# Sahar-E/NeRF-and-DietNeRF

Hardware: AMD Instinct MI355X
Metric: rays/sec (coarse+fine) at 256x256, 64 coarse + 128 fine samples (higher is better)
Workload: dtype f16 (3-pass hi/lo split operands, f32 accumulate; fp32-class results)

## Files before the change

### include/nerf_mi355.h

```cpp
#ifndef NERF_MI355_H
#define NERF_MI355_H

#include <stddef.h>
#include <stdint.h>

#ifdef __cplusplus
extern "C" {
#endif

#define NERF_ABI_VERSION 6

enum { NERF_NET_COARSE = 0, NERF_NET_FINE = 1 };
enum { NERF_MEM_HOST = 0, NERF_MEM_DEVICE = 1 };
enum {
    NERF_PRECISION_FP32 = 0,
    NERF_PRECISION_F16X3 = 1,
    NERF_PRECISION_F16 = 2,
    NERF_PRECISION_BF16X3 = 3
};

enum {
    NERF_SAMPLING_LINEAR = 0,
    NERF_SAMPLING_LINDISP = 1
};
// ... 133 lines not shown
                         uint64_t seed, float* grad_coarse, float* grad_fine, float* metrics, int mem);
int nerf_train_apply(nerf_ctx* ctx, const float* grad_coarse, const float* grad_fine, int mem);
int nerf_train_render_gradients(nerf_ctx* ctx, const float* rays_orig, const float* rays_dirs, const float* d_rgb,
                                int64_t N, int32_t Sc, int32_t Sf, const float* u_coarse, const float* u_fine,
                                uint64_t seed, int64_t ray_base, int32_t accumulate, float* rgb_out,
                                float* grad_coarse, float* grad_fine, int mem);
int nerf_train_render_forward(nerf_ctx* ctx, int32_t slot, const float* rays_orig, const float* rays_dirs, int64_t N,
                              int32_t Sc, int32_t Sf, const float* u_coarse, const float* u_fine, uint64_t seed,
                              int64_t ray_base, float* rgb_out, int mem);
int nerf_train_render_backward(nerf_ctx* ctx, int32_t slot, const float* d_rgb, int32_t accumulate, float* grad_coarse,
                               float* grad_fine, int mem);
int nerf_train_render_release(nerf_ctx* ctx);
int nerf_train_get_gradients(nerf_ctx* ctx, int which, float* blob, size_t n_floats, int mem);
int nerf_get_weights(nerf_ctx* ctx, int which, float* blob, size_t n_floats, int mem);

int nerf_ctx_enable_timing(nerf_ctx* ctx, int on);
int nerf_ctx_read_timing(nerf_ctx* ctx, double* mlp_ms, int64_t* n_launches, int64_t* n_rows);
int nerf_ctx_read_culling_timing(nerf_ctx* ctx, double* ms4, int64_t* n_passes);

#ifdef __cplusplus
}
#endif
#endif
```

### nerf_and_dietnerf_amd/_lib.py

```python
from __future__ import annotations

import ctypes as C
import os

_HERE = os.path.dirname(os.path.abspath(__file__))
LIB_PATH = os.environ.get("NERF_MI355_LIB") or os.path.join(_HERE, "lib", "libnerf_mi355.so")

NERF_NET_COARSE, NERF_NET_FINE = 0, 1
NERF_MEM_HOST, NERF_MEM_DEVICE = 0, 1
NERF_PRECISION_FP32, NERF_PRECISION_F16X3, NERF_PRECISION_F16, NERF_PRECISION_BF16X3 = 0, 1, 2, 3
NERF_SAMPLING_LINEAR, NERF_SAMPLING_LINDISP = 0, 1
NERF_RAYS_WORLD, NERF_RAYS_NDC = 0, 1
NERF_ABI_VERSION = 6


class NerfConfig(C.Structure):
    _fields_ = [
        ("n_pos_enc_xyz", C.c_int32), ("n_pos_enc_dir", C.c_int32), ("n_angles", C.c_int32),
        ("hidden_dim", C.c_int32), ("last_hidden_dim", C.c_int32), ("leaky_relu_alpha", C.c_float),
        ("near_boundary", C.c_float), ("far_boundary", C.c_float), ("precision", C.c_int32),
        ("device", C.c_int32),
    ]


# ... 65 lines not shown
    ("nerf_train_set_distortion_weights", C.c_int, [_P, _F, _F]),
    ("nerf_train_read_distortion_sums", C.c_int, [_P, C.POINTER(C.c_double), C.POINTER(_I64)]),
    ("nerf_distortion_loss", C.c_int, [_P, _P, _P, _I64, _I32, _P, _P, _P, C.c_int]),
    ("nerf_train_loss_scale", C.c_int, [_P, C.POINTER(C.c_float), C.POINTER(_I64), C.POINTER(_I64)]),
    ("nerf_train_read_metric_sums", C.c_int, [_P, C.POINTER(C.c_double), C.POINTER(_I64)]),
    ("nerf_train_step", C.c_int, [_P, _P, _P, _P, _I64, _I32, _I32, _P, _P, _U64, _P, C.c_int]),
    ("nerf_train_gradients", C.c_int, [_P, _P, _P, _P, _I64, _I32, _I32, _P, _P, _U64, _P, _P, _P, C.c_int]),
    ("nerf_train_apply", C.c_int, [_P, _P, _P, C.c_int]),
    ("nerf_train_render_gradients", C.c_int, [_P, _P, _P, _P, _I64, _I32, _I32, _P, _P, _U64, _I64, _I32, _P, _P, _P,
                                              C.c_int]),
    ("nerf_train_render_forward", C.c_int, [_P, _I32, _P, _P, _I64, _I32, _I32, _P, _P, _U64, _I64, _P, C.c_int]),
    ("nerf_train_render_backward", C.c_int, [_P, _I32, _P, _I32, _P, _P, C.c_int]),
    ("nerf_train_render_release", C.c_int, [_P]),
    ("nerf_train_get_gradients", C.c_int, [_P, C.c_int, _P, C.c_size_t, C.c_int]),
    ("nerf_get_weights", C.c_int, [_P, C.c_int, _P, C.c_size_t, C.c_int]),
    ("nerf_ctx_enable_timing", C.c_int, [_P, C.c_int]),
    ("nerf_ctx_read_timing", C.c_int, [_P, C.POINTER(C.c_double), C.POINTER(_I64), C.POINTER(_I64)]),
]

_lib = None


def load():
    global _lib
    if _lib is not None:
        return _lib
    if not os.path.exists(LIB_PATH):
        raise RuntimeError(
            f"{LIB_PATH} is missing: build the HIP extension first "
            "(python -c 'import __graft_entry__ as g; g.build()' or make -C nerf_and_dietnerf_amd/csrc). "
# ... 24 lines not shown
```

### nerf_and_dietnerf_amd/csrc/nerf_api.hip

```cpp
#include "../../include/nerf_mi355.h"

#include <stdarg.h>
#include <stdio.h>
#include <stdlib.h>
#include <string.h>

#include <algorithm>
#include <cmath>
#include <string>
#include <vector>

#include "nerf_ctx.h"

using namespace nerf;

thread_local std::string g_err;

namespace nerf {

int fail(const char* fmt, ...) {
    char buf[512];
    va_list ap;
    va_start(ap, fmt);
    vsnprintf(buf, sizeof buf, fmt, ap);
    va_end(ap);
    g_err = buf;
// ... 50 lines not shown
    return 0;
}

int enter(nerf_ctx* c) {
    if (!c) return fail("ctx is NULL");
    HIP_OK(hipSetDevice(c->cfg.device));
    return 0;
}

int sampling_ok(const nerf_ctx* c) {
    if (c->sampling == NERF_SAMPLING_LINDISP && !(c->cfg.near_boundary > 0.f)) return fail("lindisp needs near_boundary > 0");
    return 0;
}

int draw_z_values(nerf_ctx* c, const float* o, const float* d, long long N, int S, const float* u, uint64_t seed,
                  long long ray_base, float* z) {
    const float* bounds = nullptr;
    const int* state = nullptr;
    if (c->box_on && c->grid_R > 0 && o && d && N > 0) {
        if (int r = ensure(c, c->b_gbounds, (size_t)N * 8)) return r;
        if (int r = ensure(c, c->b_gstate, (size_t)N * 4)) return r;
        launch_ray_grid_bounds(c->box, c->cfg.near_boundary, c->cfg.far_boundary, (const uint32_t*)c->b_grid[c->grid_cur].p,
                               c->grid_R, o, d, N, (float*)c->b_gbounds.p, (int*)c->b_gstate.p, c->stream);
        bounds = (const float*)c->b_gbounds.p;
        state = (const int*)c->b_gstate.p;
    }
    launch_z_values(c->cfg.near_boundary, c->cfg.far_boundary, c->sampling == NERF_SAMPLING_LINDISP, N, S, u, seed, ray_base,
                    z, c->stream, o, d, c->box_on ? &c->box : nullptr, bounds, state);
    return 0;
}

static int cull_stamp(nerf_ctx* c, bool stamp = true) {
    if (!stamp || !c->timing) return 0;
    if (c->cull_ev_used == c->cull_ev.size()) {
        hipEvent_t e;
        HIP_OK(hipEventCreate(&e));
        c->cull_ev.push_back(e);
    }
    HIP_OK(hipEventRecord(c->cull_ev[c->cull_ev_used++], c->stream));
    return 0;
}

int compact_samples(nerf_ctx* c, SampleCompaction& rec, const float* o, const float* d, const float* z, long long N, int S,
// ... 112 lines not shown
    if (!cfg) return fail("nerf_config is NULL");
    if (cfg->n_angles != 2 && cfg->n_angles != 1 && cfg->n_angles != 0)
        return fail("n_angles_for_model should be 1 or 2.");
    if (cfg->n_pos_enc_xyz < 1 || cfg->n_pos_enc_xyz > kLxWide || cfg->n_pos_enc_dir < 1 || cfg->n_pos_enc_dir > kLd ||
        cfg->hidden_dim != kHidden || cfg->last_hidden_dim != kLast)
        return fail("supported networks: n_pos_enc_dim_xyz 1..%d, n_pos_enc_view_dir 1..%d, hidden %d, last hidden %d "
                    "(got %d %d %d %d)", kLxWide, kLd, kHidden, kLast, cfg->n_pos_enc_xyz, cfg->n_pos_enc_dir, cfg->hidden_dim,
                    cfg->last_hidden_dim);
    RenderKernel k;
    if (pick_render_kernel(*cfg, cfg->precision, false, &k) == 2)
        return fail("unknown precision %d (NERF_PRECISION_FP32 = 0, NERF_PRECISION_F16X3 = 1, NERF_PRECISION_F16 = 2, "
                    "NERF_PRECISION_BF16X3 = 3)", cfg->precision);
    return 0;
}

int run_mlp(nerf_ctx* c, int which, const RenderKernel& k, const float* in_a, const float* in_b, const float* z, float* raw,
            long long M, int S, int mode) {
    if (!c->net[which].loaded) return fail("network %d has no weights loaded", which);
    if (int r = train_flush_weights(c, which)) return r;
    MlpArgs a{};
    a.wstream = (const float*)c->net[which].stream[k.stream];
    a.wconst = c->net[which].cst[k.cst];
    if (!a.wstream || !a.wconst) return fail("internal: network %d keeps no stream of kind %d", which, (int)k.stream);
    a.in_a = in_a; a.in_b = in_b; a.z = z; a.raw = raw; a.M = M; a.S = S; a.mode = mode;
    a.nonfinite = c->nonfinite;
    a.alpha = c->cfg.leaky_relu_alpha;
    hipEvent_t e0 = nullptr, e1 = nullptr;
    if (c->timing) {
        if (c->ev_used == c->ev_pool.size()) {
            hipEvent_t x, y;
            HIP_OK(hipEventCreate(&x));
            HIP_OK(hipEventCreate(&y));
            c->ev_pool.emplace_back(x, y);
        }
        e0 = c->ev_pool[c->ev_used].first; e1 = c->ev_pool[c->ev_used].second;
        c->ev_used++;
        c->timed_rows += M;
        HIP_OK(hipEventRecord(e0, c->stream));
    }
    k.launch(a, c->num_cus, c->stream, c->cfg.n_angles == 0);
    if (c->timing) HIP_OK(hipEventRecord(e1, c->stream));
    HIP_OK(hipGetLastError());
    return 0;
}

struct OutSizes { size_t per_ray[7]; };
OutSizes out_sizes(int S) {
    OutSizes o;
    o.per_ray[0] = 3; o.per_ray[1] = S; o.per_ray[2] = S; o.per_ray[3] = S; o.per_ray[4] = 3 * (size_t)S;
    o.per_ray[5] = S; o.per_ray[6] = 1;
    return o;
}
float** out_ptrs(nerf_outputs& o, int i) {
    switch (i) {
        case 0: return &o.rgb; case 1: return &o.weights; case 2: return &o.cumprod; case 3: return &o.alpha;
        case 4: return &o.rgb_samples; case 5: return &o.z; default: return &o.depth;
    }
}

nerf_outputs stage_outputs(nerf_ctx* c, Staging& st, const nerf_outputs& outs, long long N, int S) {
    const OutSizes sz = out_sizes(S);
    nerf_outputs dev = outs;
    for (int i = 0; i < 7; ++i) {
        float** p = out_ptrs(dev, i);
        *p = st.out(c->b_out[i], *p, sz.per_ray[i] * N * sizeof(float));
    }
    return dev;
}

int copy_back_batch(nerf_ctx* c, const nerf_outputs* host, const nerf_outputs* dev, long long off, long long n, int S,
                    size_t batch_index) {
    if (!c->copy_stream) HIP_OK(hipStreamCreateWithFlags(&c->copy_stream, hipStreamNonBlocking));
    constexpr size_t kRing = 64;
    if (c->copy_ev.size() < kRing) {
        hipEvent_t e;
        HIP_OK(hipEventCreateWithFlags(&e, hipEventDisableTiming));
        c->copy_ev.push_back(e);
    }
    hipEvent_t ev = c->copy_ev[batch_index % c->copy_ev.size()];
    HIP_OK(hipEventRecord(ev, c->stream));
    HIP_OK(hipStreamWaitEvent(c->copy_stream, ev, 0));
    const OutSizes sz = out_sizes(S);
    nerf_outputs h = host ? *host : nerf_outputs{};
    nerf_outputs d = *dev;
    for (int i = 0; i < 7; ++i) {
        float* hp = *out_ptrs(h, i);
        if (!hp) continue;
        HIP_OK(hipMemcpyAsync(hp + sz.per_ray[i] * off, *out_ptrs(d, i) + sz.per_ray[i] * off,
                              sz.per_ray[i] * n * sizeof(float), hipMemcpyDeviceToHost, c->copy_stream));
    }
    return 0;
}

int culled_mlp(nerf_ctx* c, int which, const RenderKernel& k, const float* o, const float* d, const float* z, long long N, int S,
               float* raw) {
    if (!c->net[which].loaded) return fail("network %d has no weights loaded", which);
    if (int r = compact_samples(c, c->cull, o, d, z, N, S, true)) return r;
    const long long M = c->cull.rows;
    if (M > 0) {
        if (int r = ensure(c, c->b_craw, (size_t)M * (k.sigma_only ? 4 : 16))) return r;
        const float* view = c->cfg.n_angles != 0 ? (const float*)c->b_cdirs.p : nullptr;
        if (int r = run_mlp(c, which, k, (const float*)c->b_cxyz.p, view, nullptr, (float*)c->b_craw.p, M, 1, 1)) return r;
    }
    if (int r = cull_stamp(c)) return r;
    launch_raw_expand((const float*)c->b_craw.p, N * S, k.sigma_only, (const uint8_t*)c->cull.mask.p,
                      (const uint32_t*)c->cull.first.p, raw, c->stream);
    return cull_stamp(c);
}

int network_pass(nerf_ctx* c, int which, const RenderKernel& k, const float* o, const float* d, const float* z, long long N, int S,
                 float* raw) {
    if (!(culling_acts(c, c->cull_on) && N > 0)) return run_mlp(c, which, k, o, d, z, raw, N * S, S, 0);
    const size_t ev0 = c->cull_ev_used;
    const int r = culled_mlp(c, which, k, o, d, z, N, S, raw);
    if (r) c->cull_ev_used = ev0;
    return r;
}

int dev_render_rays(nerf_ctx* c, int which, const float* o, const float* d, const float* z, long long N, int S,
                    const nerf_outputs& outs) {
    const bool weights_only = outs.weights && !outs.rgb && !outs.cumprod && !outs.alpha && !outs.rgb_samples && !outs.z &&
                              !outs.depth;
    RenderKernel k;
    if (pick_render_kernel(c->cfg, c->cfg.precision, which == NERF_NET_COARSE && weights_only, &k)) return 1;
    if (k.sigma_only) {
        if (int r = ensure(c, c->b_raw, (size_t)N * S * sizeof(float))) return r;
        float* sigma = (float*)c->b_raw.p;
        if (int r = network_pass(c, which, k, o, d, z, N, S, sigma)) return r;
        launch_composite_weights(sigma, z, N, S, outs.weights, c->stream);
        HIP_OK(hipGetLastError());
        return 0;
    }
    if (int r = ensure(c, c->b_raw, (size_t)N * S * 4 * sizeof(float))) return r;
    float* raw = (float*)c->b_raw.p;
    if (int r = network_pass(c, which, k, o, d, z, N, S, raw)) return r;
    launch_composite(raw, z, N, S, outs.rgb, outs.weights, outs.cumprod, outs.alpha, outs.rgb_samples, outs.depth,
                     c->stream);
    if (outs.z && outs.z != z)
        HIP_OK(hipMemcpyAsync(outs.z, z, (size_t)N * S * sizeof(float), hipMemcpyDeviceToDevice, c->stream));
    HIP_OK(hipGetLastError());
    return 0;
}

int dev_render(nerf_ctx* c, const float* o, const float* d, long long N, int Sc, int Sf, const float* u_c,
               const float* u_f, uint64_t seed, long long ray_base, const nerf_outputs& outs) {
    const bool fine = Sf > 0 && c->net[NERF_NET_FINE].loaded;
    if (int r = sampling_ok(c)) return r;
    if (int r = ensure(c, c->b_zc, (size_t)N * Sc * sizeof(float))) return r;
    float* zc = (float*)c->b_zc.p;
    if (int r = draw_z_values(c, o, d, N, Sc, u_c, seed, ray_base, zc)) return r;
    if (!fine) return dev_render_rays(c, NERF_NET_COARSE, o, d, zc, N, Sc, outs);
    if (Sc < 2) return fail("hierarchical sampling needs at least 2 coarse samples (got %d)", Sc);
    if (int r = ensure(c, c->b_wc, (size_t)N * Sc * sizeof(float))) return r;
    nerf_outputs co{};
    co.weights = (float*)c->b_wc.p;
    if (int r = dev_render_rays(c, NERF_NET_COARSE, o, d, zc, N, Sc, co)) return r;
    const int St = Sc + Sf;
    if (int r = ensure(c, c->b_zf, (size_t)N * St * sizeof(float))) return r;
    float* zf = (float*)c->b_zf.p;
    launch_sample_pdf(co.weights, zc, N, Sc, Sf, u_f, seed, ray_base, nullptr, zf, c->stream);
    return dev_render_rays(c, NERF_NET_FINE, o, d, zf, N, St, outs);
}

}

extern "C" {

int nerf_abi_version(void) { return NERF_ABI_VERSION; }
const char* nerf_last_error(void) { return g_err.c_str(); }

size_t nerf_blob_size(const nerf_config* cfg) {
    if (check_cfg(cfg)) return 0;
    return blob_floats(cfg->n_pos_enc_xyz, cfg->n_pos_enc_dir, cfg->n_angles);
}

int nerf_ctx_create(const nerf_config* cfg, nerf_ctx** out) {
// ... 32 lines not shown
    bf16::wide::mlp_bf16x3_set_attributes();
    mlp_bwd_f16x3_set_attributes();
    mlp_f16_2t_set_attributes();
    *out = c;
    return 0;
}

void nerf_ctx_destroy(nerf_ctx* c) {
    if (!c) return;
    (void)hipSetDevice(c->cfg.device);
    (void)hipStreamSynchronize(c->stream);
    DevBuf* bufs[] = {&c->b_orig, &c->b_dirs, &c->b_zc, &c->b_zf, &c->b_raw, &c->b_wc, &c->b_u0, &c->b_u1,
                      &c->b_in0, &c->b_in1, &c->b_in2, &c->b_grid[0], &c->b_grid[1], &c->b_gbounds, &c->b_gstate,
                      &c->b_mesh_v, &c->b_mesh_n, &c->b_mesh_t, &c->b_mesh_sigma, &c->b_mesh_mask, &c->b_mesh_first,
                      &c->b_mesh_count, &c->b_mesh_tfirst, &c->b_mesh_sums, &c->b_lattice, &c->cull.mask, &c->cull.first,
                      &c->b_csums, &c->b_cxyz, &c->b_cdirs, &c->b_craw};
    for (DevBuf* b : bufs) if (b->p) (void)hipFree(b->p);
    for (auto& b : c->b_out) if (b.p) (void)hipFree(b.p);
    for (auto& n : c->net) {
        for (void* p : n.stream) if (p) (void)hipFree(p);
        for (float* p : n.cst) if (p) (void)hipFree(p);
        if (n.dev_blob) (void)hipFree(n.dev_blob);
    }
    for (int32_t* p : c->rt) if (p) (void)hipFree(p);
    for (int32_t* p : c->rt_cst) if (p) (void)hipFree(p);
    for (auto& ev : c->ev_pool) { (void)hipEventDestroy(ev.first); (void)hipEventDestroy(ev.second); }
    if (c->copy_stream) { (void)hipStreamSynchronize(c->copy_stream); (void)hipStreamDestroy(c->copy_stream); }
    for (hipEvent_t e : c->copy_ev) (void)hipEventDestroy(e);
    for (hipEvent_t e : c->cull_ev) (void)hipEventDestroy(e);
    if (c->cull_rows) (void)hipHostFree(c->cull_rows);
    comm_free(c);
    train_free(c);
    if (c->nonfinite) (void)hipFree(c->nonfinite);
    if (c->own_stream) (void)hipStreamDestroy(c->own_stream);
    delete c;
}

int nerf_ctx_synchronize(nerf_ctx* c) {
    if (!c) return fail("ctx is NULL");
    HIP_OK(hipStreamSynchronize(c->stream));
    return 0;
}
// ... 93 lines not shown
    const long long cells = (long long)R * R * R;
    const size_t bytes = (size_t)cells / 8;
    c->grid_R = 0;
    if (int r = ensure(c, c->b_grid[0], bytes)) return r;
    if (int r = ensure(c, c->b_grid[1], bytes)) return r;
    const long long chunk_cells = std::min(cells, (((long long)1 << 20) / samples_per_cell) & ~63LL);
    const size_t pts = (size_t)chunk_cells * samples_per_cell;
    if (int r = ensure(c, c->b_in0, pts * 12)) return r;
    if (int r = ensure(c, c->b_in1, pts * 12)) return r;
    if (int r = ensure(c, c->b_raw, pts * 16)) return r;
    float *xyz = (float*)c->b_in0.p, *view = (float*)c->b_in1.p, *raw = (float*)c->b_raw.p;
    int cur = 0;
    for (long long begin = 0; begin < cells; begin += chunk_cells) {
        const long long n = std::min(chunk_cells, cells - begin);
        launch_grid_points(c->box, R, begin, n, samples_per_cell, seed, xyz, view, c->stream);
        if (int r = run_mlp(c, which, k, xyz, c->cfg.n_angles != 0 ? view : nullptr, nullptr, raw, n * samples_per_cell, 1, 1))
            return r;
        launch_grid_threshold(raw, begin, n, samples_per_cell, sigma_threshold, (uint32_t*)c->b_grid[cur].p, c->stream);
    }
    for (int i = 0; i < dilate; ++i, cur ^= 1)
        launch_grid_dilate((const uint32_t*)c->b_grid[cur].p, (uint32_t*)c->b_grid[cur ^ 1].p, R, c->stream);
    HIP_OK(hipGetLastError());
    if (n_occupied) {
        std::vector<uint32_t> host(bytes / 4);
        HIP_OK(hipMemcpyAsync(host.data(), c->b_grid[cur].p, bytes, hipMemcpyDeviceToHost, c->stream));
        HIP_OK(hipStreamSynchronize(c->stream));
        long long count = 0;
        for (uint32_t w : host) count += __builtin_popcount(w);
        *n_occupied = count;
    }
    c->grid_cur = cur;
// ... 14 lines not shown
    if (pick_render_kernel(c->cfg, c->cfg.precision, false, &k)) return 1;
    const float up[3] = {0.f, 0.f, 1.f};
    const float* vd = view_dir3 ? view_dir3 : up;
    const long long points = (long long)n * n * n;
    const size_t pts = (size_t)std::min(points, kMeshChunk);
    if (int r = ensure(c, c->b_in0, pts * 12)) return r;
    if (int r = ensure(c, c->b_in1, pts * 12)) return r;
    if (int r = ensure(c, c->b_raw, pts * 16)) return r;
    Staging st(c, mem);
    float* out = st.out(c->b_lattice, sigma, (size_t)points * 4);
    if (st.err) return st.err;
    float *xyz = (float*)c->b_in0.p, *view = c->cfg.n_angles != 0 ? (float*)c->b_in1.p : nullptr, *raw = (float*)c->b_raw.p;
    for (long long begin = 0; begin < points; begin += kMeshChunk) {
        const long long m = std::min(kMeshChunk, points - begin);
        launch_lattice_points(c->box, n, begin, m, vd, xyz, view, c->stream);
        if (int r = run_mlp(c, which, k, xyz, view, nullptr, raw, m, 1, 1)) return r;
        launch_raw_sigma(raw, m, out + begin, c->stream);
    }
    HIP_OK(hipGetLastError());
    return st.finish();
}

int nerf_mesh_colors(nerf_ctx* c, int which, const float* vertices, const float* normals, int64_t V, float* rgb, int mem) {
    ENTER(c);
    if (V < 0) return fail("bad V");
    if (V == 0) return 0;
    if (!vertices || !normals || !rgb) return fail("NULL argument");
    if (which != 0 && which != 1) return fail("which must be 0 (coarse) or 1 (fine)");
    if (!c->net[which].loaded) return fail("network %d has no weights loaded", which);
    RenderKernel k;
    if (pick_render_kernel(c->cfg, c->cfg.precision, false, &k)) return 1;
    const size_t pts = (size_t)std::min((long long)V, kMeshChunk);
    if (int r = ensure(c, c->b_in1, pts * 12)) return r;
    if (int r = ensure(c, c->b_raw, pts * 16)) return r;
    float *view = (float*)c->b_in1.p, *raw = (float*)c->b_raw.p;
    for (long long begin = 0; begin < V; begin += kMeshChunk) {
        const long long m = std::min(kMeshChunk, (long long)V - begin);
        Staging st(c, mem);
        const float* xyz = st.in(c->b_in0, vertices + 3 * begin, (size_t)m * 12);
        const float* nrm = st.in(c->b_in2, normals + 3 * begin, (size_t)m * 12);
        float* out = st.out(c->b_out[0], rgb + 3 * begin, (size_t)m * 12);
        if (st.err) return st.err;
        launch_mesh_view(nrm, m, view, c->stream);
        if (int r = run_mlp(c, which, k, xyz, c->cfg.n_angles != 0 ? view : nullptr, nullptr, raw, m, 1, 1)) return r;
        launch_raw_rgb(raw, m, out, c->stream);
        HIP_OK(hipGetLastError());
        if (int r = st.finish()) return r;
    }
    return 0;
}

int nerf_ctx_set_precision(nerf_ctx* c, int precision) {
    if (!c) return fail("ctx is NULL");
    RenderKernel k;
    if (pick_render_kernel(c->cfg, precision, false, &k)) return 1;
    HIP_OK(hipStreamSynchronize(c->stream));
    c->cfg.precision = precision;
    return 0;
}
// ... 206 lines not shown
}

int nerf_model_predict(nerf_ctx* c, int which, const float* xyz, const float* view_dirs, int64_t M, float* raw,
                       int mem) {
    ENTER(c);
    if (!c || !xyz || !raw || (!view_dirs && c->cfg.n_angles != 0)) return fail("NULL argument");
    if (which != 0 && which != 1) return fail("which must be 0 (coarse) or 1 (fine)");
    if (M < 0) return fail("bad M");
    Staging st(c, mem);
    const float* dx = st.in(c->b_in0, xyz, (size_t)M * 12);
    const float* dv = st.in(c->b_in1, view_dirs, (size_t)M * 12);
    float* dr = st.out(c->b_raw, raw, (size_t)M * 16);
    if (st.err) return st.err;
    RenderKernel k;
    if (pick_render_kernel(c->cfg, c->cfg.precision, false, &k)) return 1;
    if (int r = run_mlp(c, which, k, dx, dv, nullptr, dr, M, 1, 1)) return r;
    return st.finish();
}

int nerf_ray_marching(nerf_ctx* c, const float* raw, const float* z, int64_t N, int32_t S, const nerf_outputs* outs,
                      int mem) {
    ENTER(c);
    if (!c || !raw || !z || !outs) return fail("NULL argument");
    if (N < 0 || S <= 0) return fail("bad shape");
    Staging st(c, mem);
    const float* dr = st.in(c->b_raw, raw, (size_t)N * S * 16);
    const float* dz = st.in(c->b_zc, z, (size_t)N * S * 4);
    const nerf_outputs dev = stage_outputs(c, st, *outs, N, S);
    if (st.err) return st.err;
    launch_composite(dr, dz, N, S, dev.rgb, dev.weights, dev.cumprod, dev.alpha, dev.rgb_samples, dev.depth, c->stream);
    if (dev.z && dev.z != dz) HIP_OK(hipMemcpyAsync(dev.z, dz, (size_t)N * S * 4, hipMemcpyDeviceToDevice, c->stream));
// ... 1 lines not shown
    return st.finish();
}

int nerf_render_rays(nerf_ctx* c, int which, const float* o, const float* d, const float* z, int64_t N, int32_t S,
                     const nerf_outputs* outs, int mem) {
    ENTER(c);
    if (!c || !o || !d || !z || !outs) return fail("NULL argument");
    if (which != 0 && which != 1) return fail("which must be 0 (coarse) or 1 (fine)");
    if (N < 0 || S <= 0) return fail("bad shape");
    Staging st(c, mem);
    const float* so = st.in(c->b_orig, o, (size_t)N * 16);
    const float* sd = st.in(c->b_dirs, d, (size_t)N * 16);
    const float* sz = st.in(c->b_zc, z, (size_t)N * S * 4);
    const nerf_outputs dev = stage_outputs(c, st, *outs, N, S);
    if (st.err) return st.err;
    if (int r = dev_render_rays(c, which, so, sd, sz, N, S, dev)) return r;
    return st.finish();
}

int nerf_render(nerf_ctx* c, const float* o, const float* d, int64_t N, int32_t Sc, int32_t Sf, const float* u_c,
                const float* u_f, uint64_t seed, int64_t ray_base, const nerf_outputs* outs, int mem) {
    ENTER(c);
    if (!c || !o || !d || !outs) return fail("NULL argument");
    if (N < 0 || Sc <= 0 || Sf < 0) return fail("bad shape N=%lld Sc=%d Sf=%d", (long long)N, Sc, Sf);
    const bool fine = Sf > 0 && c->net[NERF_NET_FINE].loaded;
    const int S = fine ? Sc + Sf : Sc;
    if (fine && sample_pdf_lds_bytes(Sc, Sf) > 64 * 1024) return fail("Sc=%d Sf=%d exceeds the sampler's LDS budget", Sc, Sf);
    Staging st(c, mem);
    const float* so = st.in(c->b_orig, o, (size_t)N * 16);
    const float* sd = st.in(c->b_dirs, d, (size_t)N * 16);
    const float* duc = st.in(c->b_u0, u_c, (size_t)N * Sc * 4);
    const float* duf = st.in(c->b_u1, fine ? u_f : nullptr, (size_t)N * Sf * 4);
    const nerf_outputs dev = stage_outputs(c, st, *outs, N, S);
    if (st.err) return st.err;
    if (int r = dev_render(c, so, sd, N, Sc, Sf, duc, duf, seed, ray_base, dev)) return r;
    return st.finish();
}

int nerf_render_image(nerf_ctx* c, const float* c2w, float fov, int32_t H, int32_t W, int64_t ray_begin,
                      int64_t ray_count, int64_t batch, int32_t Sc, int32_t Sf, const float* u_c, const float* u_f,
                      uint64_t seed, const nerf_outputs* outs, int mem) {
    ENTER(c);
    if (!c || !c2w || !outs) return fail("NULL argument");
    if (H <= 0 || W <= 0 || Sc <= 0 || Sf < 0) return fail("bad shape");
    const long long total = (long long)H * W;
    if (ray_count <= 0) { ray_begin = 0; ray_count = total; }
    if (ray_begin < 0 || ray_begin + ray_count > total) return fail("ray slab [%lld,+%lld) outside %lld rays",
                                                                    (long long)ray_begin, (long long)ray_count, total);
    if (batch < 0) return fail("batch_size must be > 0");
    const bool fine = Sf > 0 && c->net[NERF_NET_FINE].loaded;
    const int S = fine ? Sc + Sf : Sc;
    if (fine && sample_pdf_lds_bytes(Sc, Sf) > 64 * 1024) return fail("Sc=%d Sf=%d exceeds the sampler's LDS budget", Sc, Sf);
    const long long N = ray_count;
    if (int r = sampling_ok(c)) return r;
    if (batch == 0) {
        batch = 1 << 18;
        const bool per_sample = outs->weights || outs->cumprod || outs->alpha || outs->rgb_samples || outs->z;
        if (mem == NERF_MEM_HOST && per_sample && N >= 32768) batch = ((N + 3) / 4 + 127) / 128 * 128;
    }
    if (int r = ensure(c, c->b_orig, (size_t)N * 16)) return r;
    if (int r = ensure(c, c->b_dirs, (size_t)N * 16)) return r;
    launch_raygen(c2w, fov, H, W, ray_begin, N, (float*)c->b_orig.p, (float*)c->b_dirs.p, c->stream);
    if (c->ray_space == NERF_RAYS_NDC)
        launch_rays_to_ndc((const float*)c->b_orig.p, (const float*)c->b_dirs.p, N, fov, c->ndc_near_plane, (float*)c->b_orig.p,
                           (float*)c->b_dirs.p, c->stream);
    const float *duc = u_c, *duf = u_f;
    nerf_outputs dev = *outs;
    if (mem == NERF_MEM_HOST) {
        if (u_c) { if (int r = h2d(c, c->b_u0, u_c + ray_begin * Sc, (size_t)N * Sc * 4)) return r; duc = (const float*)c->b_u0.p; }
        if (u_f && fine) { if (int r = h2d(c, c->b_u1, u_f + ray_begin * Sf, (size_t)N * Sf * 4)) return r; duf = (const float*)c->b_u1.p; }
        Staging st(c, mem);
        dev = stage_outputs(c, st, *outs, N, S);
        if (st.err) return st.err;
    } else {
        if (u_c) duc = u_c + ray_begin * Sc;
        if (u_f) duf = u_f + ray_begin * Sf;
    }
    const OutSizes sz = out_sizes(S);
    size_t k = 0;
    for (long long off = 0; off < N; off += batch, ++k) {
        const long long n = std::min<long long>(batch, N - off);
        nerf_outputs part = dev;
        for (int i = 0; i < 7; ++i) {
            float** p = out_ptrs(part, i);
            if (*p) *p += sz.per_ray[i] * off;
        }
        if (int r = dev_render(c, (const float*)c->b_orig.p + off * 4, (const float*)c->b_dirs.p + off * 4, n, Sc, Sf,
                               duc ? duc + off * Sc : nullptr, (duf && fine) ? duf + off * Sf : nullptr, seed,
                               ray_begin + off, part)) {
            if (c->copy_stream) (void)hipStreamSynchronize(c->copy_stream);
            return r;
        }
        if (mem == NERF_MEM_HOST)
            if (int r = copy_back_batch(c, outs, &dev, off, n, S, k)) { (void)hipStreamSynchronize(c->copy_stream); return r; }
    }
    if (mem == NERF_MEM_HOST && c->copy_stream) HIP_OK(hipStreamSynchronize(c->copy_stream));
    return 0;
}

int nerf_host_alloc(size_t bytes, void** out) {
    if (!out) return fail("out is NULL");
    *out = nullptr;
    if (bytes == 0) return fail("nerf_host_alloc of 0 bytes");
    HIP_OK(hipHostMalloc(out, bytes, hipHostMallocPortable));
    return 0;
}

int nerf_host_free(void* p) {
    if (!p) return 0;
    HIP_OK(hipHostFree(p));
    return 0;
// ... 43 lines not shown
```

### nerf_and_dietnerf_amd/csrc/nerf_ctx.h

```cpp
#pragma once
#include "../../include/nerf_mi355.h"

#include <string>
#include <utility>
#include <vector>

#include "nerf_kernels.h"

namespace nerf {

int fail(const char* fmt, ...);

#define HIP_OK(expr)                                                                                    \
    do {                                                                                                \
        hipError_t e__ = (expr);                                                                        \
        if (e__ != hipSuccess) return nerf::fail("%s failed: %s (%s:%d)", #expr, hipGetErrorString(e__), \
                                                 __FILE__, __LINE__);                                   \
    } while (0)

struct DevBuf {
    void* p = nullptr;
    size_t cap = 0;
};

struct NetWeights {
    void* stream[kStreamKinds] = {};
    float* cst[kConstBlocks] = {};
    bool loaded = false;
    std::vector<float> host_blob;
    float* dev_blob = nullptr;
};

struct SampleCompaction { DevBuf mask, first; long long rows = -1; };

struct TrainState;
struct CommState;

}

struct nerf_ctx {
    nerf_config cfg;
    int sampling = NERF_SAMPLING_LINEAR;
    int ray_space = NERF_RAYS_WORLD;
    float ndc_near_plane = 1.0f;
    bool box_on = false;
    nerf::SceneBox box = {};
    int grid_R = 0;
    int grid_cur = 0;
// ... 12 lines not shown
    long long mesh_V = 0, mesh_T = 0;
    nerf::DevBuf b_mesh_v, b_mesh_n, b_mesh_t;
    nerf::DevBuf b_mesh_sigma, b_mesh_mask, b_mesh_first, b_mesh_count, b_mesh_tfirst, b_mesh_sums;
    nerf::DevBuf b_lattice;
    int num_cus = 0;
    hipStream_t own_stream = nullptr;
    hipStream_t stream = nullptr;
    hipStream_t copy_stream = nullptr;
    std::vector<hipEvent_t> copy_ev;
    nerf::NetWeights net[2];
    int32_t* rt[nerf::kStreamKinds] = {};
    int32_t* rt_cst[nerf::kConstBlocks] = {};
    bool rt_built = false;
    nerf::DevBuf b_orig, b_dirs, b_zc, b_zf, b_raw, b_wc, b_u0, b_u1, b_in0, b_in1, b_in2;
    nerf::DevBuf b_out[7];
    bool timing = false;
    std::vector<std::pair<hipEvent_t, hipEvent_t>> ev_pool;
    size_t ev_used = 0;
    long long timed_rows = 0;
    unsigned long long* nonfinite = nullptr;
    nerf::TrainState* train = nullptr;
    nerf::CommState* comm = nullptr;
};

namespace nerf {

int ensure(nerf_ctx* c, DevBuf& b, size_t bytes);
int h2d(nerf_ctx* c, DevBuf& b, const void* src, size_t bytes);
int enter(nerf_ctx* c);
int copy_to_caller(nerf_ctx* c, void* dst, const void* src_dev, size_t bytes, int mem);
// ... 4 lines not shown
    template <class T> const T* in(DevBuf& b, const T* src, size_t bytes) { return (const T*)stage(b, (void*)src, bytes, true); }
    template <class T> T* out(DevBuf& b, T* dst, size_t bytes) { return (T*)stage(b, dst, bytes, false); }
    int finish();
    int err = 0;

private:
    void* stage(DevBuf& b, void* caller, size_t bytes, bool upload);
    nerf_ctx* c;
    bool host;
    struct { void* dst; const void* src; size_t bytes; } back[7];
    int n_back = 0;
};
#define ENTER(c) do { if (int r__ = nerf::enter(c)) return r__; } while (0)
int sampling_ok(const nerf_ctx* c);
int draw_z_values(nerf_ctx* c, const float* o, const float* d, long long N, int S, const float* u, uint64_t seed,
                   long long ray_base, float* z);

inline bool culling_acts(const nerf_ctx* c, bool flag) { return flag && c->box_on && c->grid_R > 0; }
int compact_samples(nerf_ctx* c, SampleCompaction& rec, const float* o, const float* d, const float* z, long long N, int S,
                    bool stamp);

void train_free(nerf_ctx* c);
void comm_free(nerf_ctx* c);
int comm_allreduce_mean(nerf_ctx* c, float* buf, size_t n);
int comm_world(const nerf_ctx* c);
int ensure_render_tables(nerf_ctx* c);
int repack_render_streams(nerf_ctx* c, int which, const float* dev_blob);
int train_on_load(nerf_ctx* c, int which);
int train_flush_weights(nerf_ctx* c, int which, bool to_host = false);

}
// ... 1 lines not shown
```

### nerf_and_dietnerf_amd/render.py

```python
from __future__ import annotations

import ctypes as C
from typing import Dict, List, Optional, Sequence, Tuple

import numpy as np

from . import _lib
from ._lib import (NerfTrainConfig, NERF_MEM_DEVICE, NERF_MEM_HOST, NERF_NET_COARSE, NERF_NET_FINE, NERF_PRECISION_F16X3,
                   NERF_PRECISION_FP32, NerfConfig, NerfOutputs)

N_RENDER_SAMPLES_FINE = "n_render_samples_fine"
N_RENDER_SAMPLES_COARSE = "n_render_samples_coarse"
N_POS_ENC_DIM_XYZ = "n_pos_enc_dim_xyz"
N_POS_ENC_VIEW_DIR = "n_pos_enc_view_dir"
N_ANGLES_FOR_MODEL = "n_angles_for_model"
LEAKY_RELU_ALPHA = "leaky_relu_alpha"
HIDDEN_LAYER_DIM = "hidden_layer_dim"
LAST_HIDDEN_LAYER_DIM = "last_hidden_layer_dim"
N_RAYS_IN_BATCH_RENDER = "n_rays_in_batch_render"
N_RAYS_IN_BATCH_TRAIN = "n_rays_in_batch_train"
LINDISP = "lindisp"
USE_NDC = "use_ndc"
NDC_NEAR_PLANE = "ndc_near_plane"
SCENE_BOX = "scene_box"
# ... 205 lines not shown
        _lib.check(self.lib.nerf_ctx_create(C.byref(self.cfg), C.byref(h)))
        self.h = h
        self.loaded = [False, False]
        self._stream = None
        self.comm_world = 0
        self.precision = precision
        self._auto_fp32 = False
        self._auto_unchecked = False
        self.auto_fallbacks = 0
        self._slot_fine = {}
        self.sampling, self.ray_space, self.ndc_near_plane = "linear", "world", 1.0
        self.scene_box = None
        self.grid_resolution = 0
        self.sample_culling = False
        self._train_sample_culling = False

    def close(self):
        if getattr(self, "h", None):
            self.lib.nerf_ctx_destroy(self.h)
            self.h = None

    def __del__(self):
        try:
            self.close()
        except Exception:
            pass

    def blob_size(self) -> int:
        return int(self.lib.nerf_blob_size(C.byref(self.cfg)))

# ... 451 lines not shown
    def train_apply(self, grad_coarse=None, grad_fine=None) -> None:
        arr = self._arrays(grad_coarse, grad_fine)
        n = self.blob_size()
        _lib.check(self.lib.nerf_train_apply(self.h, arr.inp(grad_coarse, (n,)), arr.inp(grad_fine, (n,)), arr.mem))
        self._auto_new_weights()

    def train_get_gradients(self, which: int) -> np.ndarray:
        out = np.empty(self.blob_size(), np.float32)
        _lib.check(self.lib.nerf_train_get_gradients(self.h, which, out.ctypes.data, out.size, NERF_MEM_HOST))
        return out

    def get_weights(self, which: int) -> np.ndarray:
        out = np.empty(self.blob_size(), np.float32)
        _lib.check(self.lib.nerf_get_weights(self.h, which, out.ctypes.data, out.size, NERF_MEM_HOST))
        return out

    def enable_timing(self, on: bool = True) -> None:
        _lib.check(self.lib.nerf_ctx_enable_timing(self.h, int(on)))

    def read_timing(self) -> Tuple[float, int, int]:
        ms, n, rows = C.c_double(), C.c_int64(), C.c_int64()
        _lib.check(self.lib.nerf_ctx_read_timing(self.h, C.byref(ms), C.byref(n), C.byref(rows)))
        return ms.value, n.value, rows.value

    def _arrays(self, *probe) -> "_Arrays":
        arr = _Arrays(*probe)
        if arr.torch is not None:
            cur = arr.torch.cuda.current_stream(arr.device).cuda_stream
            if cur != self._stream:
                _lib.check(self.lib.nerf_ctx_set_stream(self.h, C.c_void_p(cur)))
# ... 463 lines not shown
```

Measured before the change: 1.789 million.

## Split render batches across two streams to overlap coarse/fine pipeline stages

Adds a second stream (lane) with its own scratch buffers and splits a single render batch into up to four tile-aligned pieces that alternate between the context stream and the lane stream, using fork/join events. The intent is to overlap the coarse MLP, PDF sampling and fine MLP of one piece with another so the GPU stays fuller and per-piece serial gaps are hidden. It costs extra device memory for the duplicate buffers and smaller per-launch work, and it falls back to one lane when culling is active or allocation fails.

Result: no change. 1.793 million (median of 6 runs) (+0.3%).

```diff
diff --git a/include/nerf_mi355.h b/include/nerf_mi355.h
--- a/include/nerf_mi355.h
+++ b/include/nerf_mi355.h
@@ -171,6 +171,8 @@
 int nerf_train_get_gradients(nerf_ctx* ctx, int which, float* blob, size_t n_floats, int mem);
 int nerf_get_weights(nerf_ctx* ctx, int which, float* blob, size_t n_floats, int mem);
 
+int nerf_ctx_set_batches_in_flight(nerf_ctx* ctx, int n, int64_t min_split_rays);
+
 int nerf_ctx_enable_timing(nerf_ctx* ctx, int on);
 int nerf_ctx_read_timing(nerf_ctx* ctx, double* mlp_ms, int64_t* n_launches, int64_t* n_rows);
 int nerf_ctx_read_culling_timing(nerf_ctx* ctx, double* ms4, int64_t* n_passes);
diff --git a/nerf_and_dietnerf_amd/_lib.py b/nerf_and_dietnerf_amd/_lib.py
--- a/nerf_and_dietnerf_amd/_lib.py
+++ b/nerf_and_dietnerf_amd/_lib.py
@@ -103,6 +103,7 @@
     ("nerf_train_render_release", C.c_int, [_P]),
     ("nerf_train_get_gradients", C.c_int, [_P, C.c_int, _P, C.c_size_t, C.c_int]),
     ("nerf_get_weights", C.c_int, [_P, C.c_int, _P, C.c_size_t, C.c_int]),
+    ("nerf_ctx_set_batches_in_flight", C.c_int, [_P, C.c_int, _I64]),
     ("nerf_ctx_enable_timing", C.c_int, [_P, C.c_int]),
     ("nerf_ctx_read_timing", C.c_int, [_P, C.POINTER(C.c_double), C.POINTER(_I64), C.POINTER(_I64)]),
 ]
diff --git a/nerf_and_dietnerf_amd/csrc/batch_plan.h b/nerf_and_dietnerf_amd/csrc/batch_plan.h
--- /dev/null
+++ b/nerf_and_dietnerf_amd/csrc/batch_plan.h
@@ -0,0 +1,33 @@
+#pragma once
+#include <algorithm>
+#include <vector>
+
+namespace nerf {
+
+struct BatchPiece { long long off, n; };
+
+constexpr long long kOwnBatch = 1LL << 18;
+constexpr int kTileRows = 128;
+constexpr int kMinTilesPerWorkgroup = 16;
+
+inline long long split_threshold(int Sc, int num_cus, int pieces) {
+    const long long rows = (long long)pieces * kMinTilesPerWorkgroup * kTileRows * std::max(num_cus, 1);
+    return (rows + std::max(Sc, 1) - 1) / std::max(Sc, 1);
+}
+
+inline std::vector<BatchPiece> plan_batches(long long N, long long batch, int in_flight, int Sc, int num_cus,
+                                            long long min_split_rays = -1, int pieces = 4) {
+    std::vector<BatchPiece> out;
+    if (N <= 0) return out;
+    const bool own = batch <= 0;
+    if (own) batch = kOwnBatch;
+    if (own && in_flight >= 2 && N <= batch) {
+        int p = min_split_rays < 0 ? pieces : (N >= min_split_rays ? 2 : 1);
+        if (min_split_rays < 0) while (p >= 2 && N < split_threshold(Sc, num_cus, p)) p /= 2;
+        if (p >= 2) batch = ((N + p - 1) / p + kTileRows - 1) / kTileRows * kTileRows;
+    }
+    for (long long off = 0; off < N; off += batch) out.push_back({off, std::min(batch, N - off)});
+    return out;
+}
+
+}
diff --git a/nerf_and_dietnerf_amd/csrc/nerf_api.hip b/nerf_and_dietnerf_amd/csrc/nerf_api.hip
--- a/nerf_and_dietnerf_amd/csrc/nerf_api.hip
+++ b/nerf_and_dietnerf_amd/csrc/nerf_api.hip
@@ -10,6 +10,7 @@
 #include <string>
 #include <vector>
 
+#include "batch_plan.h"
 #include "nerf_ctx.h"
 
 using namespace nerf;
@@ -90,19 +91,20 @@
 }
 
 int draw_z_values(nerf_ctx* c, const float* o, const float* d, long long N, int S, const float* u, uint64_t seed,
-                  long long ray_base, float* z) {
+                  long long ray_base, float* z, const Lane* lane) {
+    const Lane l = lane ? *lane : lane0(c);
     const float* bounds = nullptr;
     const int* state = nullptr;
     if (c->box_on && c->grid_R > 0 && o && d && N > 0) {
-        if (int r = ensure(c, c->b_gbounds, (size_t)N * 8)) return r;
-        if (int r = ensure(c, c->b_gstate, (size_t)N * 4)) return r;
+        if (int r = ensure(c, *l.gbounds, (size_t)N * 8)) return r;
+        if (int r = ensure(c, *l.gstate, (size_t)N * 4)) return r;
         launch_ray_grid_bounds(c->box, c->cfg.near_boundary, c->cfg.far_boundary, (const uint32_t*)c->b_grid[c->grid_cur].p,
-                               c->grid_R, o, d, N, (float*)c->b_gbounds.p, (int*)c->b_gstate.p, c->stream);
-        bounds = (const float*)c->b_gbounds.p;
-        state = (const int*)c->b_gstate.p;
+                               c->grid_R, o, d, N, (float*)l.gbounds->p, (int*)l.gstate->p, l.stream);
+        bounds = (const float*)l.gbounds->p;
+        state = (const int*)l.gstate->p;
     }
     launch_z_values(c->cfg.near_boundary, c->cfg.far_boundary, c->sampling == NERF_SAMPLING_LINDISP, N, S, u, seed, ray_base,
-                    z, c->stream, o, d, c->box_on ? &c->box : nullptr, bounds, state);
+                    z, l.stream, o, d, c->box_on ? &c->box : nullptr, bounds, state);
     return 0;
 }
 
@@ -245,8 +247,8 @@
     return 0;
 }
 
-int run_mlp(nerf_ctx* c, int which, const RenderKernel& k, const float* in_a, const float* in_b, const float* z, float* raw,
-            long long M, int S, int mode) {
+int run_mlp(nerf_ctx* c, hipStream_t s, int which, const RenderKernel& k, const float* in_a, const float* in_b, const float* z,
+            float* raw, long long M, int S, int mode) {
     if (!c->net[which].loaded) return fail("network %d has no weights loaded", which);
     if (int r = train_flush_weights(c, which)) return r;
     MlpArgs a{};
@@ -267,10 +269,10 @@
         e0 = c->ev_pool[c->ev_used].first; e1 = c->ev_pool[c->ev_used].second;
         c->ev_used++;
         c->timed_rows += M;
-        HIP_OK(hipEventRecord(e0, c->stream));
-    }
-    k.launch(a, c->num_cus, c->stream, c->cfg.n_angles == 0);
-    if (c->timing) HIP_OK(hipEventRecord(e1, c->stream));
+        HIP_OK(hipEventRecord(e0, s));
+    }
+    k.launch(a, c->num_cus, s, c->cfg.n_angles == 0);
+    if (c->timing) HIP_OK(hipEventRecord(e1, s));
     HIP_OK(hipGetLastError());
     return 0;
 }
@@ -299,8 +301,8 @@
     return dev;
 }
 
-int copy_back_batch(nerf_ctx* c, const nerf_outputs* host, const nerf_outputs* dev, long long off, long long n, int S,
-                    size_t batch_index) {
+int copy_back_batch(nerf_ctx* c, hipStream_t producer, const nerf_outputs* host, const nerf_outputs* dev, long long off,
+                    long long n, int S, size_t batch_index) {
     if (!c->copy_stream) HIP_OK(hipStreamCreateWithFlags(&c->copy_stream, hipStreamNonBlocking));
     constexpr size_t kRing = 64;
     if (c->copy_ev.size() < kRing) {
@@ -309,7 +311,7 @@
         c->copy_ev.push_back(e);
     }
     hipEvent_t ev = c->copy_ev[batch_index % c->copy_ev.size()];
-    HIP_OK(hipEventRecord(ev, c->stream));
+    HIP_OK(hipEventRecord(ev, producer));
     HIP_OK(hipStreamWaitEvent(c->copy_stream, ev, 0));
     const OutSizes sz = out_sizes(S);
     nerf_outputs h = host ? *host : nerf_outputs{};
@@ -331,7 +333,7 @@
     if (M > 0) {
         if (int r = ensure(c, c->b_craw, (size_t)M * (k.sigma_only ? 4 : 16))) return r;
         const float* view = c->cfg.n_angles != 0 ? (const float*)c->b_cdirs.p : nullptr;
-        if (int r = run_mlp(c, which, k, (const float*)c->b_cxyz.p, view, nullptr, (float*)c->b_craw.p, M, 1, 1)) return r;
+        if (int r = run_mlp(c, c->stream, which, k, (const float*)c->b_cxyz.p, view, nullptr, (float*)c->b_craw.p, M, 1, 1)) return r;
     }
     if (int r = cull_stamp(c)) return r;
     launch_raw_expand((const float*)c->b_craw.p, N * S, k.sigma_only, (const uint8_t*)c->cull.mask.p,
@@ -339,58 +341,85 @@
     return cull_stamp(c);
 }
 
-int network_pass(nerf_ctx* c, int which, const RenderKernel& k, const float* o, const float* d, const float* z, long long N, int S,
-                 float* raw) {
-    if (!(culling_acts(c, c->cull_on) && N > 0)) return run_mlp(c, which, k, o, d, z, raw, N * S, S, 0);
+int network_pass(nerf_ctx* c, const Lane& l, int which, const RenderKernel& k, const float* o, const float* d, const float* z,
+                 long long N, int S, float* raw) {
+    if (!(culling_acts(c, c->cull_on) && N > 0)) return run_mlp(c, l.stream, which, k, o, d, z, raw, N * S, S, 0);
+    if (l.stream != c->stream) return fail("internal: a culled pass off the ctx stream");
     const size_t ev0 = c->cull_ev_used;
     const int r = culled_mlp(c, which, k, o, d, z, N, S, raw);
     if (r) c->cull_ev_used = ev0;
     return r;
 }
 
-int dev_render_rays(nerf_ctx* c, int which, const float* o, const float* d, const float* z, long long N, int S,
+int dev_render_rays(nerf_ctx* c, const Lane& l, int which, const float* o, const float* d, const float* z, long long N, int S,
                     const nerf_outputs& outs) {
     const bool weights_only = outs.weights && !outs.rgb && !outs.cumprod && !outs.alpha && !outs.rgb_samples && !outs.z &&
                               !outs.depth;
     RenderKernel k;
     if (pick_render_kernel(c->cfg, c->cfg.precision, which == NERF_NET_COARSE && weights_only, &k)) return 1;
     if (k.sigma_only) {
-        if (int r = ensure(c, c->b_raw, (size_t)N * S * sizeof(float))) return r;
-        float* sigma = (float*)c->b_raw.p;
-        if (int r = network_pass(c, which, k, o, d, z, N, S, sigma)) return r;
-        launch_composite_weights(sigma, z, N, S, outs.weights, c->stream);
+        if (int r = ensure(c, *l.raw, (size_t)N * S * sizeof(float))) return r;
+        float* sigma = (float*)l.raw->p;
+        if (int r = network_pass(c, l, which, k, o, d, z, N, S, sigma)) return r;
+        launch_composite_weights(sigma, z, N, S, outs.weights, l.stream);
         HIP_OK(hipGetLastError());
         return 0;
     }
-    if (int r = ensure(c, c->b_raw, (size_t)N * S * 4 * sizeof(float))) return r;
-    float* raw = (float*)c->b_raw.p;
-    if (int r = network_pass(c, which, k, o, d, z, N, S, raw)) return r;
+    if (int r = ensure(c, *l.raw, (size_t)N * S * 4 * sizeof(float))) return r;
+    float* raw = (float*)l.raw->p;
+    if (int r = network_pass(c, l, which, k, o, d, z, N, S, raw)) return r;
     launch_composite(raw, z, N, S, outs.rgb, outs.weights, outs.cumprod, outs.alpha, outs.rgb_samples, outs.depth,
-                     c->stream);
+                     l.stream);
     if (outs.z && outs.z != z)
-        HIP_OK(hipMemcpyAsync(outs.z, z, (size_t)N * S * sizeof(float), hipMemcpyDeviceToDevice, c->stream));
-    HIP_OK(hipGetLastError());
-    return 0;
-}
-
-int dev_render(nerf_ctx* c, const float* o, const float* d, long long N, int Sc, int Sf, const float* u_c,
+        HIP_OK(hipMemcpyAsync(outs.z, z, (size_t)N * S * sizeof(float), hipMemcpyDeviceToDevice, l.stream));
+    HIP_OK(hipGetLastError());
+    return 0;
+}
+
+int dev_render(nerf_ctx* c, const Lane& l, const float* o, const float* d, long long N, int Sc, int Sf, const float* u_c,
                const float* u_f, uint64_t seed, long long ray_base, const nerf_outputs& outs) {
     const bool fine = Sf > 0 && c->net[NERF_NET_FINE].loaded;
     if (int r = sampling_ok(c)) return r;
-    if (int r = ensure(c, c->b_zc, (size_t)N * Sc * sizeof(float))) return r;
-    float* zc = (float*)c->b_zc.p;
-    if (int r = draw_z_values(c, o, d, N, Sc, u_c, seed, ray_base, zc)) return r;
-    if (!fine) return dev_render_rays(c, NERF_NET_COARSE, o, d, zc, N, Sc, outs);
+    if (int r = ensure(c, *l.zc, (size_t)N * Sc * sizeof(float))) return r;
+    float* zc = (float*)l.zc->p;
+    if (int r = draw_z_values(c, o, d, N, Sc, u_c, seed, ray_base, zc, &l)) return r;
+    if (!fine) return dev_render_rays(c, l, NERF_NET_COARSE, o, d, zc, N, Sc, outs);
     if (Sc < 2) return fail("hierarchical sampling needs at least 2 coarse samples (got %d)", Sc);
-    if (int r = ensure(c, c->b_wc, (size_t)N * Sc * sizeof(float))) return r;
+    if (int r = ensure(c, *l.wc, (size_t)N * Sc * sizeof(float))) return r;
     nerf_outputs co{};
-    co.weights = (float*)c->b_wc.p;
-    if (int r = dev_render_rays(c, NERF_NET_COARSE, o, d, zc, N, Sc, co)) return r;
+    co.weights = (float*)l.wc->p;
+    if (int r = dev_render_rays(c, l, NERF_NET_COARSE, o, d, zc, N, Sc, co)) return r;
     const int St = Sc + Sf;
-    if (int r = ensure(c, c->b_zf, (size_t)N * St * sizeof(float))) return r;
-    float* zf = (float*)c->b_zf.p;
-    launch_sample_pdf(co.weights, zc, N, Sc, Sf, u_f, seed, ray_base, nullptr, zf, c->stream);
-    return dev_render_rays(c, NERF_NET_FINE, o, d, zf, N, St, outs);
+    if (int r = ensure(c, *l.zf, (size_t)N * St * sizeof(float))) return r;
+    float* zf = (float*)l.zf->p;
+    launch_sample_pdf(co.weights, zc, N, Sc, Sf, u_f, seed, ray_base, nullptr, zf, l.stream);
+    return dev_render_rays(c, l, NERF_NET_FINE, o, d, zf, N, St, outs);
+}
+
+bool prepare_lanes(nerf_ctx* c, long long n0, long long n1, int Sc, int Sf, bool fine, Lane* lane1) {
+    if (!c->lane_stream && hipStreamCreateWithFlags(&c->lane_stream, hipStreamNonBlocking) != hipSuccess) {
+        c->lane_stream = nullptr;
+        (void)hipGetLastError();
+        return false;
+    }
+    if (!c->fork_ev && hipEventCreateWithFlags(&c->fork_ev, hipEventDisableTiming) != hipSuccess) { c->fork_ev = nullptr; return false; }
+    if (!c->join_ev && hipEventCreateWithFlags(&c->join_ev, hipEventDisableTiming) != hipSuccess) { c->join_ev = nullptr; return false; }
+    const Lane l0 = lane0(c);
+    *lane1 = {c->lane_stream, &c->l1_zc, &c->l1_wc, &c->l1_zf, &c->l1_raw, &c->l1_gbounds, &c->l1_gstate};
+    const bool grid = c->box_on && c->grid_R > 0;
+    const size_t St = fine ? (size_t)Sc + Sf : (size_t)Sc;
+    const size_t raw_per_ray = St * 4 * sizeof(float);
+    const Lane* lanes[2] = {&l0, lane1};
+    const long long rays[2] = {n0, n1};
+    for (int i = 0; i < 2; ++i) {
+        const Lane& l = *lanes[i];
+        const size_t n = (size_t)rays[i];
+        bool ok = !ensure(c, *l.zc, n * Sc * sizeof(float)) && !ensure(c, *l.raw, n * raw_per_ray);
+        if (ok && fine) ok = !ensure(c, *l.wc, n * Sc * sizeof(float)) && !ensure(c, *l.zf, n * St * sizeof(float));
+        if (ok && grid) ok = !ensure(c, *l.gbounds, n * 8) && !ensure(c, *l.gstate, n * 4);
+        if (!ok) { (void)hipGetLastError(); return false; }
+    }
+    return true;
 }
 
 }
@@ -453,7 +482,8 @@
                       &c->b_in0, &c->b_in1, &c->b_in2, &c->b_grid[0], &c->b_grid[1], &c->b_gbounds, &c->b_gstate,
                       &c->b_mesh_v, &c->b_mesh_n, &c->b_mesh_t, &c->b_mesh_sigma, &c->b_mesh_mask, &c->b_mesh_first,
                       &c->b_mesh_count, &c->b_mesh_tfirst, &c->b_mesh_sums, &c->b_lattice, &c->cull.mask, &c->cull.first,
-                      &c->b_csums, &c->b_cxyz, &c->b_cdirs, &c->b_craw};
+                      &c->b_csums, &c->b_cxyz, &c->b_cdirs, &c->b_craw, &c->l1_zc, &c->l1_wc, &c->l1_zf, &c->l1_raw, &c->l1_gbounds,
+                      &c->l1_gstate};
     for (DevBuf* b : bufs) if (b->p) (void)hipFree(b->p);
     for (auto& b : c->b_out) if (b.p) (void)hipFree(b.p);
     for (auto& n : c->net) {
@@ -465,6 +495,9 @@
     for (int32_t* p : c->rt_cst) if (p) (void)hipFree(p);
     for (auto& ev : c->ev_pool) { (void)hipEventDestroy(ev.first); (void)hipEventDestroy(ev.second); }
     if (c->copy_stream) { (void)hipStreamSynchronize(c->copy_stream); (void)hipStreamDestroy(c->copy_stream); }
+    if (c->lane_stream) { (void)hipStreamSynchronize(c->lane_stream); (void)hipStreamDestroy(c->lane_stream); }
+    if (c->fork_ev) (void)hipEventDestroy(c->fork_ev);
+    if (c->join_ev) (void)hipEventDestroy(c->join_ev);
     for (hipEvent_t e : c->copy_ev) (void)hipEventDestroy(e);
     for (hipEvent_t e : c->cull_ev) (void)hipEventDestroy(e);
     if (c->cull_rows) (void)hipHostFree(c->cull_rows);
@@ -588,7 +621,7 @@
     for (long long begin = 0; begin < cells; begin += chunk_cells) {
         const long long n = std::min(chunk_cells, cells - begin);
         launch_grid_points(c->box, R, begin, n, samples_per_cell, seed, xyz, view, c->stream);
-        if (int r = run_mlp(c, which, k, xyz, c->cfg.n_angles != 0 ? view : nullptr, nullptr, raw, n * samples_per_cell, 1, 1))
+        if (int r = run_mlp(c, c->stream, which, k, xyz, c->cfg.n_angles != 0 ? view : nullptr, nullptr, raw, n * samples_per_cell, 1, 1))
             return r;
         launch_grid_threshold(raw, begin, n, samples_per_cell, sigma_threshold, (uint32_t*)c->b_grid[cur].p, c->stream);
     }
@@ -633,7 +666,7 @@
     for (long long begin = 0; begin < points; begin += kMeshChunk) {
         const long long m = std::min(kMeshChunk, points - begin);
         launch_lattice_points(c->box, n, begin, m, vd, xyz, view, c->stream);
-        if (int r = run_mlp(c, which, k, xyz, view, nullptr, raw, m, 1, 1)) return r;
+        if (int r = run_mlp(c, c->stream, which, k, xyz, view, nullptr, raw, m, 1, 1)) return r;
         launch_raw_sigma(raw, m, out + begin, c->stream);
     }
     HIP_OK(hipGetLastError());
@@ -661,7 +694,7 @@
         float* out = st.out(c->b_out[0], rgb + 3 * begin, (size_t)m * 12);
         if (st.err) return st.err;
         launch_mesh_view(nrm, m, view, c->stream);
-        if (int r = run_mlp(c, which, k, xyz, c->cfg.n_angles != 0 ? view : nullptr, nullptr, raw, m, 1, 1)) return r;
+        if (int r = run_mlp(c, c->stream, which, k, xyz, c->cfg.n_angles != 0 ? view : nullptr, nullptr, raw, m, 1, 1)) return r;
         launch_raw_rgb(raw, m, out, c->stream);
         HIP_OK(hipGetLastError());
         if (int r = st.finish()) return r;
@@ -898,7 +931,7 @@
     if (st.err) return st.err;
     RenderKernel k;
     if (pick_render_kernel(c->cfg, c->cfg.precision, false, &k)) return 1;
-    if (int r = run_mlp(c, which, k, dx, dv, nullptr, dr, M, 1, 1)) return r;
+    if (int r = run_mlp(c, c->stream, which, k, dx, dv, nullptr, dr, M, 1, 1)) return r;
     return st.finish();
 }
 
@@ -930,7 +963,7 @@
     const float* sz = st.in(c->b_zc, z, (size_t)N * S * 4);
     const nerf_outputs dev = stage_outputs(c, st, *outs, N, S);
     if (st.err) return st.err;
-    if (int r = dev_render_rays(c, which, so, sd, sz, N, S, dev)) return r;
+    if (int r = dev_render_rays(c, lane0(c), which, so, sd, sz, N, S, dev)) return r;
     return st.finish();
 }
 
@@ -949,7 +982,7 @@
     const float* duf = st.in(c->b_u1, fine ? u_f : nullptr, (size_t)N * Sf * 4);
     const nerf_outputs dev = stage_outputs(c, st, *outs, N, S);
     if (st.err) return st.err;
-    if (int r = dev_render(c, so, sd, N, Sc, Sf, duc, duf, seed, ray_base, dev)) return r;
+    if (int r = dev_render(c, lane0(c), so, sd, N, Sc, Sf, duc, duf, seed, ray_base, dev)) return r;
     return st.finish();
 }
 
@@ -970,9 +1003,21 @@
     const long long N = ray_count;
     if (int r = sampling_ok(c)) return r;
     if (batch == 0) {
-        batch = 1 << 18;
         const bool per_sample = outs->weights || outs->cumprod || outs->alpha || outs->rgb_samples || outs->z;
         if (mem == NERF_MEM_HOST && per_sample && N >= 32768) batch = ((N + 3) / 4 + 127) / 128 * 128;
+    }
+    const int in_flight = culling_acts(c, c->cull_on) ? 1 : c->in_flight;
+    std::vector<BatchPiece> plan = plan_batches(N, batch, in_flight, Sc, c->num_cus, c->min_split_rays);
+    Lane lanes[2] = {lane0(c), lane0(c)};
+    bool two = in_flight >= 2 && plan.size() > 1;
+    if (two) {
+        long long most[2] = {0, 0};
+        for (size_t i = 0; i < plan.size(); ++i) most[i & 1] = std::max(most[i & 1], plan[i].n);
+        two = prepare_lanes(c, most[0], most[1], Sc, Sf, fine, &lanes[1]);
+        if (!two) {
+            lanes[1] = lanes[0];
+            plan = plan_batches(N, batch, 1, Sc, c->num_cus);
+        }
     }
     if (int r = ensure(c, c->b_orig, (size_t)N * 16)) return r;
     if (int r = ensure(c, c->b_dirs, (size_t)N * 16)) return r;
@@ -993,24 +1038,48 @@
         if (u_f) duf = u_f + ray_begin * Sf;
     }
     const OutSizes sz = out_sizes(S);
-    size_t k = 0;
-    for (long long off = 0; off < N; off += batch, ++k) {
-        const long long n = std::min<long long>(batch, N - off);
+    if (two) {
+        if (int r = train_flush_weights(c, NERF_NET_COARSE)) return r;
+        if (fine) if (int r = train_flush_weights(c, NERF_NET_FINE)) return r;
+        HIP_OK(hipGetLastError());
+        HIP_OK(hipEventRecord(c->fork_ev, c->stream));
+        HIP_OK(hipStreamWaitEvent(c->lane_stream, c->fork_ev, 0));
+    }
+    auto join = [&]() -> int {
+        if (!two) return 0;
+        HIP_OK(hipEventRecord(c->join_ev, c->lane_stream));
+        HIP_OK(hipStreamWaitEvent(c->stream, c->join_ev, 0));
+        return 0;
+    };
+    for (size_t k = 0; k < plan.size(); ++k) {
+        const long long off = plan[k].off, n = plan[k].n;
+        const Lane& l = lanes[k & 1];
         nerf_outputs part = dev;
         for (int i = 0; i < 7; ++i) {
             float** p = out_ptrs(part, i);
             if (*p) *p += sz.per_ray[i] * off;
         }
-        if (int r = dev_render(c, (const float*)c->b_orig.p + off * 4, (const float*)c->b_dirs.p + off * 4, n, Sc, Sf,
-                               duc ? duc + off * Sc : nullptr, (duf && fine) ? duf + off * Sf : nullptr, seed,
-                               ray_begin + off, part)) {
+        int r = dev_render(c, l, (const float*)c->b_orig.p + off * 4, (const float*)c->b_dirs.p + off * 4, n, Sc, Sf,
+                           duc ? duc + off * Sc : nullptr, (duf && fine) ? duf + off * Sf : nullptr, seed, ray_begin + off, part);
+        if (!r && mem == NERF_MEM_HOST) r = copy_back_batch(c, l.stream, outs, &dev, off, n, S, k);
+        if (r) {
+            const std::string why = g_err;
+            (void)join();
+            g_err = why;
             if (c->copy_stream) (void)hipStreamSynchronize(c->copy_stream);
             return r;
         }
-        if (mem == NERF_MEM_HOST)
-            if (int r = copy_back_batch(c, outs, &dev, off, n, S, k)) { (void)hipStreamSynchronize(c->copy_stream); return r; }
-    }
+    }
+    if (int r = join()) return r;
     if (mem == NERF_MEM_HOST && c->copy_stream) HIP_OK(hipStreamSynchronize(c->copy_stream));
+    return 0;
+}
+
+int nerf_ctx_set_batches_in_flight(nerf_ctx* c, int n, int64_t min_split_rays) {
+    if (!c) return fail("ctx is NULL");
+    if (n != 1 && n != 2) return fail("batches in flight: n must be 1 or 2 (got %d)", n);
+    c->in_flight = n;
+    c->min_split_rays = min_split_rays < 0 ? -1 : (long long)min_split_rays;
     return 0;
 }
 
diff --git a/nerf_and_dietnerf_amd/csrc/nerf_ctx.h b/nerf_and_dietnerf_amd/csrc/nerf_ctx.h
--- a/nerf_and_dietnerf_amd/csrc/nerf_ctx.h
+++ b/nerf_and_dietnerf_amd/csrc/nerf_ctx.h
@@ -32,6 +32,11 @@
 };
 
 struct SampleCompaction { DevBuf mask, first; long long rows = -1; };
+
+struct Lane {
+    hipStream_t stream;
+    DevBuf *zc, *wc, *zf, *raw, *gbounds, *gstate;
+};
 
 struct TrainState;
 struct CommState;
@@ -74,6 +79,11 @@
     bool rt_built = false;
     nerf::DevBuf b_orig, b_dirs, b_zc, b_zf, b_raw, b_wc, b_u0, b_u1, b_in0, b_in1, b_in2;
     nerf::DevBuf b_out[7];
+    int in_flight = 2;
+    long long min_split_rays = -1;
+    hipStream_t lane_stream = nullptr;
+    hipEvent_t fork_ev = nullptr, join_ev = nullptr;
+    nerf::DevBuf l1_zc, l1_wc, l1_zf, l1_raw, l1_gbounds, l1_gstate;
     bool timing = false;
     std::vector<std::pair<hipEvent_t, hipEvent_t>> ev_pool;
     size_t ev_used = 0;
@@ -108,7 +118,8 @@
 #define ENTER(c) do { if (int r__ = nerf::enter(c)) return r__; } while (0)
 int sampling_ok(const nerf_ctx* c);
 int draw_z_values(nerf_ctx* c, const float* o, const float* d, long long N, int S, const float* u, uint64_t seed,
-                   long long ray_base, float* z);
+                   long long ray_base, float* z, const Lane* lane = nullptr);
+inline Lane lane0(nerf_ctx* c) { return {c->stream, &c->b_zc, &c->b_wc, &c->b_zf, &c->b_raw, &c->b_gbounds, &c->b_gstate}; }
 
 inline bool culling_acts(const nerf_ctx* c, bool flag) { return flag && c->box_on && c->grid_R > 0; }
 int compact_samples(nerf_ctx* c, SampleCompaction& rec, const float* o, const float* d, const float* z, long long N, int S,
diff --git a/nerf_and_dietnerf_amd/render.py b/nerf_and_dietnerf_amd/render.py
--- a/nerf_and_dietnerf_amd/render.py
+++ b/nerf_and_dietnerf_amd/render.py
@@ -1,6 +1,7 @@
 from __future__ import annotations
 
 import ctypes as C
+import os
 from typing import Dict, List, Optional, Sequence, Tuple
 
 import numpy as np
@@ -243,6 +244,9 @@
         self.grid_resolution = 0
         self.sample_culling = False
         self._train_sample_culling = False
+        self._one_lane_env = os.environ.get("NERF_BATCHES_IN_FLIGHT") == "1"
+        if self._one_lane_env:
+            self.set_batches_in_flight(1)
 
     def close(self):
         if getattr(self, "h", None):
@@ -724,6 +728,11 @@
         out = np.empty(self.blob_size(), np.float32)
         _lib.check(self.lib.nerf_get_weights(self.h, which, out.ctypes.data, out.size, NERF_MEM_HOST))
         return out
+
+    def set_batches_in_flight(self, n: int = 2, min_split_rays: int = -1) -> None:
+        if n not in (1, 2):
+            raise RuntimeError(f"batches in flight: n must be 1 or 2 (got {n})")
+        _lib.check(self.lib.nerf_ctx_set_batches_in_flight(self.h, 1 if self._one_lane_env else int(n), int(min_split_rays)))
 
     def enable_timing(self, on: bool = True) -> None:
         _lib.check(self.lib.nerf_ctx_enable_timing(self.h, int(on)))
```
